# Xinglab/abPOA

Hardware: AMD Instinct MI355X
Metric: read-sets/sec (consensus bit-exact) + DP Gcells/sec (roofline.dp_gcells_per_s) (higher is better)
Workload: dtype int16

## Files before the change

### abpoa_amd/csrc/msa_device.cpp

```cpp
#include <algorithm>
#include <atomic>
#include <chrono>
#include <limits.h>
#include <mutex>
#include <stdio.h>
#include <stdlib.h>
#include <string.h>
#include <thread>
#include <vector>
#include <hip/hip_runtime.h>
#include "engine_options.h"
#include "batch_stream.h"
#include "msa_device.h"
#include "poa_device.h"
#include "poa_graph.h"
#include "dir_plane.h"
#include "msa_batch.h"
#include "msa_device_debug.h"
#include "msa_device_plan.h"
#include "routing.h"

namespace abpoa_hip {

namespace {
// ... 277 lines not shown
    b.left = p.scratch; b.right = p.scratch;
    if (gen_io) {
        b.out_off = p.out_off; b.out_row = p.out_row; b.left = (int32_t *)(dr + L.o_left); b.right = (int32_t *)(dr + L.o_right); b.row_active = dr + L.o_act;
    }
    b.dp_beg_sn = (int32_t *)(dr + L.o_bsn); b.dp_end_sn = (int32_t *)(dr + L.o_esn); b.row_cell_off = (int64_t *)(dr + L.o_coff);
    b.row_max_i = (int32_t *)(dr + L.o_rmi);
    b.planes = C.planes.dev; b.cigar = p.cigar;
    b_rc = b;
    if (pl.amb) {
        b.want_lr = (sc->wb >= 0 && !pl.general) ? 1 : 0;
        b_rc = b; b_rc.want_lr = 0; b_rc.fresh_band = sc->wb >= 0 ? 0 : 1;
    }
    return 0;
}

void plan_rounds(Job &J) {
    const DevicePlan &pl = J.pl; const abpoa_hip_scoring_t *sc = &pl.sc; const PoaDev &p = J.p; const DevBatch &b = J.b; DevBatch &b_r = J.b_r;
    bool &dbg_sync = J.dbg_sync, &use_rounds = J.use_rounds; size_t &rounds_lds = J.rounds_lds;
    dbg_sync = opt_on("ABPOA_HIP_DEVSYNC");
    use_rounds = !pl.local && pl.rounds_possible && !dbg_sync && b.lds.wide_on == 0 && !(b.dbg & 64) && pl.max_reads > 2 && !opt_on("ABPOA_HIP_LOCKSTEP");
    b_r = b; rounds_lds = 0;
    if (use_rounds) {
        auto dyn_of = [&](const DevBatch &x) { return std::max<size_t>(std::max<size_t>((size_t)x.lds.total_rows, (size_t)x.lds.total_tail),
                (size_t)5 * (size_t)(p.lds_rows > 0 ? p.lds_rows : 0)); };
        rounds_lds = dyn_of(b_r);
        int st_lds = 0; int nb = poa_rounds_residency(sc->gap_mode, rounds_lds, &st_lds);
        if (nb < 4 && J.n_sets > nb * 256) {
            const int budget = 160 * 1024 / 4 - st_lds - 512, excess = (int)rounds_lds - budget;
            if (excess > 0 && (size_t)b_r.lds.total_tail == rounds_lds && b_r.lds.bt_bytes_tail - ((excess + 15) & ~15) >= 8 * 1024) {
                b_r.lds.bt_bytes_tail -= (excess + 15) & ~15; b_r.lds.total_tail -= (excess + 15) & ~15;
                rounds_lds = dyn_of(b_r); nb = poa_rounds_residency(sc->gap_mode, rounds_lds, &st_lds);
            }
        }
        b_r.lds.te_on = 0;
        if (b_r.dir_mode && sc->gap_mode != ABPOA_HIP_LINEAR_GAP && !opt_on("ABPOA_HIP_LATE_TAIL")) {
            const int avail = (int)rounds_lds - b_r.lds.phase_off, tables = (SPEC_WK - 1) * SPEC_PM_ROWS * 4;
            const int ring = (b_r.lds.total_rows - b_r.lds.phase_off + 15) & ~15;
            int w_ = ((avail - tables) / SPEC_WK) & ~15, m_ = w_;
            if (w_ < ring) { m_ = ring; w_ = ((avail - tables - m_) / (SPEC_WK - 1)) & ~15; }
            if (w_ >= SPEC_EARLY_MIN) { b_r.lds.te_on = 1; b_r.lds.te_main = m_; b_r.lds.te_w = w_; }
        }
        const int n_cu = device_cu_count(J.device);
        if (nb < 1 || J.n_sets > nb * n_cu) use_rounds = false;
        if (opt_set("ABPOA_HIP_VERBOSE")) fprintf(stderr,
                "[abpoa-hip] all-rounds kernel: %s, %zu B dynamic + %d B static LDS per workgroup, %d workgroups per CU, " "backtrack window %d B, helpers %s (%d + 3 x %d B)\n",
                use_rounds ? "on" : "off", rounds_lds, st_lds, nb, b_r.lds.bt_bytes_tail, b_r.lds.te_on ? "under the row loop" : "after the row loop", b_r.lds.te_main, b_r.lds.te_w);
    }
}

int queue_job(Job &J, DeviceDebug &dbg) {
    const DevicePlan &pl = J.pl; Cache &C = *J.C; const Layout &L = J.L; PoaDev &p = J.p; const DevBatch &b = J.b;
    hipStream_t st = C.stream; uint8_t *hi = C.in.host, *hg = C.graph.host, *dg = C.graph.dev, *dr = C.rows.dev; int rc;
    const int64_t *roff = (const int64_t *)(hi + L.o_roff);
    auto stage = [&](const char *what, int k) { return dbg.stage(what, k); };
    if (pl.gen_io()) HIP_OK(hipMemsetAsync(dr + L.o_act, 1, (size_t)pl.node_tot, st), ABPOA_HIP_ELAUNCH);
    if (pl.amb) HIP_OK(hipMemsetAsync(dg + L.o_isrc, 0, (size_t)pl.tot_reads, st), ABPOA_HIP_ELAUNCH);
    J.t_queue = now_s();
    HIP_OK(hipEventRecord(C.ev[0], st), ABPOA_HIP_ELAUNCH);
    if (stage("upload", 0)) return ABPOA_HIP_ELAUNCH;
    HIP_OK(launch_poa_init(p, st), ABPOA_HIP_ELAUNCH);
    if (stage("init", 0)) return ABPOA_HIP_ELAUNCH;
    dbg.graph_check(0);
    HIP_OK(hipEventRecord(C.ev[1], st), ABPOA_HIP_ELAUNCH);
    for (int k = 1; k < pl.max_reads; ++k) {
        if (k == 2 && !J.rest_up) {
            stage_reads(J, 2, pl.max_reads);
            HIP_OK(hipMemcpyAsync(C.in.dev + L.o_reads + (size_t)J.split_at, hi + L.o_reads + (size_t)J.split_at, (size_t)(roff[pl.tot_reads] - J.split_at),
                    hipMemcpyHostToDevice, C.copy_stream), ABPOA_HIP_ELAUNCH);
            HIP_OK(hipEventRecord(C.ev_copy, C.copy_stream), ABPOA_HIP_ELAUNCH);
            HIP_OK(hipStreamWaitEvent(st, C.ev_copy, 0), ABPOA_HIP_ELAUNCH);
            J.rest_up = true;
        }
        if (J.use_rounds && k == 2) {
            HIP_OK(hipEventRecord(C.ev[2], st), ABPOA_HIP_ELAUNCH);
            HIP_OK(launch_poa_rounds(p, J.b_r, (int32_t *)(dr + L.o_ticket), C.in.host + L.o_rargs, J.slot, 2, J.rounds_lds, st), ABPOA_HIP_ELAUNCH);
            HIP_OK(hipEventRecord(C.ev[3], st), ABPOA_HIP_ELAUNCH);
            break;
        }
        p.round = k;
        hipEvent_t *e = C.ev.data() + 4 * k;
        if (p.order_mode) { HIP_OK(launch_poa_order(p, st), ABPOA_HIP_ELAUNCH); if (stage("row order", k)) return ABPOA_HIP_ELAUNCH; dbg.order_check(k); }
        HIP_OK(launch_poa_prepare(p, st), ABPOA_HIP_ELAUNCH);
        if (stage("prepare", k)) return ABPOA_HIP_ELAUNCH;
        HIP_OK(hipEventRecord(e[0], st), ABPOA_HIP_ELAUNCH);
        if (pl.general) { HIP_OK(launch_dp_general(b, st), ABPOA_HIP_ELAUNCH); HIP_OK(hipEventRecord(e[1], st), ABPOA_HIP_ELAUNCH); }
        else HIP_OK(launch_dp_fast(b, st, e[1]), ABPOA_HIP_ELAUNCH);
        if (stage("dp rows + tail", k)) return ABPOA_HIP_ELAUNCH;
        if (pl.amb) {
            HIP_OK(launch_poa_strand_check(p, st), ABPOA_HIP_ELAUNCH);
            HIP_OK(launch_dp_general(J.b_rc, st), ABPOA_HIP_ELAUNCH);
            HIP_OK(launch_poa_strand_pick(p, st), ABPOA_HIP_ELAUNCH);
            if (stage("strand retry", k)) return ABPOA_HIP_ELAUNCH;
        }
        dbg.balance_report(k, b, e[0], e[1]);
        HIP_OK(hipEventRecord(e[2], st), ABPOA_HIP_ELAUNCH);
        HIP_OK(launch_poa_fuse(p, st), ABPOA_HIP_ELAUNCH);
        if (stage("fuse", k)) return ABPOA_HIP_ELAUNCH;
        dbg.graph_check(k);
        HIP_OK(hipEventRecord(e[3], st), ABPOA_HIP_ELAUNCH);
    }
    if (pl.want_cons) { HIP_OK(launch_poa_consensus(p, st), ABPOA_HIP_ELAUNCH); if (stage("consensus", pl.max_reads)) return ABPOA_HIP_ELAUNCH; }
    if (pl.want_msa) { HIP_OK(launch_poa_msa_rank(p, st), ABPOA_HIP_ELAUNCH); if (stage("msa rank", pl.max_reads)) return ABPOA_HIP_ELAUNCH; }
    HIP_OK(hipMemcpyAsync(hg, dg, J.dl_bytes, hipMemcpyDeviceToHost, st), ABPOA_HIP_ELAUNCH);
    HIP_OK(hipStreamSynchronize(st), ABPOA_HIP_ELAUNCH);
    int64_t msa_total = 0;
    if (pl.want_msa) {
        const PoaState *hs_ = (const PoaState *)(hg + L.o_state);
        J.msa_off.resize(J.n_sets);
        for (int s = 0; s < J.n_sets; ++s) { J.msa_off[s] = msa_total; if (hs_[s].status == POA_ST_OK && hs_[s].n_nodes > 2) msa_total += (int64_t)(J.sets[s].n_reads
                + (pl.want_cons ? 1 : 0)) * std::max(0, hs_[s].msa_len); }
        if (msa_total > 0) {
            if ((rc = C.msa.need_dev((size_t)msa_total)) || (rc = C.msa.need_host((size_t)msa_total))) return rc;
            memcpy(hi + L.o_msaoff_h, J.msa_off.data(), 8 * (size_t)J.n_sets);
            HIP_OK(hipMemcpyAsync(dg + L.o_msaoff, hi + L.o_msaoff_h, 8 * (size_t)J.n_sets, hipMemcpyHostToDevice, st), ABPOA_HIP_ELAUNCH);
            p.msa_out = C.msa.dev;
            HIP_OK(launch_poa_msa_fill(p, st), ABPOA_HIP_ELAUNCH);
            if (stage("msa fill", pl.max_reads)) return ABPOA_HIP_ELAUNCH;
            HIP_OK(hipMemcpyAsync(C.msa.host, C.msa.dev, (size_t)msa_total, hipMemcpyDeviceToHost, st), ABPOA_HIP_ELAUNCH);
            HIP_OK(hipStreamSynchronize(st), ABPOA_HIP_ELAUNCH);
        }
    }
    J.t_done = now_s();
    return 0;
}

void fill_stats(const Job &J, DeviceRunStats *stats) {
    const DevicePlan &pl = J.pl; Cache &C = *J.C; const Layout &L = J.L; const PoaDev &p = J.p;
    if (opt_set("ABPOA_HIP_ORDER_PROF") && p.order_mode) {
        const PoaState *hs_ = (const PoaState *)(C.graph.host + L.o_state); double a_[4] = {0, 0, 0, 0};
        for (int s = 0; s < J.n_sets; ++s) for (int i = 0; i < 4; ++i) a_[i] += (double)hs_[s].t_phase[i];
        fprintf(stderr, "[abpoa-hip] order walk per set: %.0f single-node passes x %.0f ticks, %.0f parallel passes x %.0f ticks\n", a_[2] / J.n_sets,
                a_[2] > 0 ? a_[0] / a_[2] : 0.0, a_[3] / J.n_sets, a_[3] > 0 ? a_[1] / a_[3] : 0.0);
    }
    if (!stats) return;
    float ms = 0;
    hipEvent_t prev = C.ev[1];
    for (int k = 1; k < (J.use_rounds ? 2 : pl.max_reads); ++k) {
        hipEvent_t *e = C.ev.data() + 4 * k;
        (void)hipEventElapsedTime(&ms, prev, e[0]); stats->prepare_ms += ms;
        (void)hipEventElapsedTime(&ms, e[0], e[1]); stats->rows_ms += ms;
        (void)hipEventElapsedTime(&ms, e[1], e[2]); stats->tail_ms += ms;
        (void)hipEventElapsedTime(&ms, e[2], e[3]); stats->fuse_ms += ms;
        prev = e[3];
    }
    if (J.use_rounds) {
        (void)hipEventElapsedTime(&ms, C.ev[2], C.ev[3]); stats->rounds_ms = ms; stats->rounds_launches = 1;
        const PoaState *hs_ = (const PoaState *)(C.graph.host + L.o_state);
        double tp[4] = {0, 0, 0, 0}, tmax = 0; for (int s = 0; s < J.n_sets; ++s) { double t_ = 0;
                if (hs_[s].status == POA_ST_OK) stats->rounds_algo_bytes += hs_[s].algo_bytes - hs_[s].algo_bytes_before;
        for (int i = 0; i < 4; ++i) { tp[i] += (double)hs_[s].t_phase[i]; t_ += (double)hs_[s].t_phase[i]; } tmax = std::max(tmax, t_); }
        const double tall = tp[0] + tp[1] + tp[2] + tp[3];
        if (tall > 0) { stats->prepare_ms += ms * tp[0] / tall; stats->rows_ms += ms * tp[1] / tall; stats->tail_ms += ms * tp[2] / tall;
                stats->fuse_ms += ms * tp[3] / tall;
                        for (int i = 0; i < 4; ++i) stats->rounds_mticks[i] = tp[i] / J.n_sets * 1e-6; stats->rounds_rows_share = tp[1] / tall;
                        stats->rounds_mean_over_max = J.n_sets > 0 && tmax > 0 ? tall / J.n_sets / tmax : 0; }
        if (opt_set("ABPOA_HIP_VERBOSE") && J.n_sets > 0 && tall > 0) {
            static const char *const ph_[4] = {"prepare", "rows", "backtrack", "fuse"};
            std::vector<double> v_((size_t)J.n_sets);
            for (int i = 0; i < 4; ++i) {
                for (int s = 0; s < J.n_sets; ++s) v_[s] = (double)hs_[s].t_phase[i];
                std::sort(v_.begin(), v_.end());
                fprintf(stderr, "[abpoa-hip] all-rounds kernel, M ticks per set, %-9s: mean %.3f  p99 %.3f  max %.3f\n", ph_[i], tp[i] / J.n_sets * 1e-6,
                        v_[(size_t)std::min<long long>(J.n_sets - 1, (long long)J.n_sets * 99 / 100)] * 1e-6, v_[(size_t)J.n_sets - 1] * 1e-6);
            }
            fprintf(stderr, "[abpoa-hip] all-rounds kernel, set totals: mean %.3f M ticks, max %.3f M ticks, max / mean %.3f\n", tall / J.n_sets * 1e-6, tmax * 1e-6,
                    tmax / (tall / J.n_sets));
// ... 120 lines not shown
```

### abpoa_amd/csrc/msa_device_debug.cpp

```cpp
#include <algorithm>
#include <limits.h>
#include <stdio.h>
#include <stdlib.h>
#include <string.h>
#include "engine_options.h"
#include "msa_device_debug.h"

namespace abpoa_hip {

void consensus_flat(int n, const int32_t *order, const uint8_t *base, const uint8_t *nout, const int32_t *out_id, const int32_t *out_w,
                    const int32_t *n_read, std::vector<int> *ids, std::vector<uint8_t> *bases, std::vector<int> *cov, std::vector<int> &score,
                            std::vector<int> &max_out, int out_cap) {
    ids->clear(); bases->clear(); cov->clear();
    if (n <= 2) return;
    score.assign(n, 0); max_out.assign(n, -1);
    for (int r = n - 1; r >= 0; --r) {
        const int cur = order[r];
        const int32_t *oi = out_id + (size_t)cur * out_cap, *ow = out_w + (size_t)cur * out_cap; const int no = nout[cur];
        if (cur == 1) { max_out[cur] = -1; score[cur] = 0; }
        else if (cur == 0) {
            int path_score = -1, path_max_w = -1, max_id = -1;
            for (int i = 0; i < no; ++i) if (ow[i] > path_max_w || (ow[i] == path_max_w && score[oi[i]] > path_score)) { max_id = oi[i]; path_score =
                    score[oi[i]]; path_max_w = ow[i]; }
            max_out[cur] = max_id;
        } else {
            int max_w = INT_MIN, max_id = -1;
            for (int i = 0; i < no; ++i) {
                if (max_w < ow[i]) { max_w = ow[i]; max_id = oi[i]; }
                else if (max_w == ow[i] && score[max_id] <= score[oi[i]]) max_id = oi[i];
            }
            score[cur] = max_w + score[max_id]; max_out[cur] = max_id;
        }
    }
    for (int cur = max_out[0]; cur != 1 && cur >= 0; cur = max_out[cur]) { ids->push_back(cur); bases->push_back(base[cur]); cov->push_back(n_read[cur]); }
}

DeviceDebug::DeviceDebug(const PoaDev *p, const std::vector<PoaSet> *ps, const abpoa_hip_readset_t *sets, int n_sets, int m, int aln_cap, int max_reads,
        bool want_msa,
                         bool amb, hipStream_t stream)
    : p_(p), ps_(ps), sets_(sets), n_sets_(n_sets), m_(m), aln_cap_(aln_cap), max_reads_(max_reads), want_msa_(want_msa), amb_(amb), st_(stream) {
    on_ = opt_on("ABPOA_HIP_DEVSYNC");
    if (on_) { graphs_.resize(std::min(n_sets, 4)); for (size_t i = 0; i < graphs_.size(); ++i) graphs_[i].reset(sets[i].n_reads, want_msa); }
}

int DeviceDebug::stage(const char *what, int k) {
    if (!on_) return 0;
    fprintf(stderr, "[poa-device] round %d: %s queued\n", k, what); fflush(stderr);
    hipError_t e_ = hipStreamSynchronize(st_);
    fprintf(stderr, "[poa-device] round %d: %s -> %s\n", k, what, hipGetErrorString(e_)); fflush(stderr);
    return e_ == hipSuccess ? 0 : 1;
}

void DeviceDebug::order_check(int k) {
    if (!on_) return;
    const PoaDev &p = *p_; const std::vector<PoaSet> &ps = *ps_; const abpoa_hip_readset_t *sets = sets_; const int n_sets = n_sets_, aln_cap = aln_cap_,
            max_reads = max_reads_; const bool amb = amb_;
    std::vector<PoaGraph> &dbg_graphs = graphs_; (void)n_sets; (void)aln_cap; (void)max_reads; (void)amb; (void)ps; (void)sets;
    for (int s = 0; s < (int)dbg_graphs.size(); ++s) {
        if (k >= sets[s].n_reads) continue;
        PoaState hst; (void)hipMemcpy(&hst, (uint8_t *)p.state + sizeof(PoaState) * s, sizeof(hst), hipMemcpyDeviceToHost);
        if (hst.status != POA_ST_OK) { fprintf(stderr, "[poa-device]   set %d round %d: row order: set not ok (status %d reason %d)\n", s, k, hst.status,
                hst.reason); continue; }
        const int n = hst.n_nodes; std::vector<int32_t> order(n), row(n);
        (void)hipMemcpy(order.data(), p.row_node[hst.order_buf] + ps[s].node0, 4 * (size_t)n, hipMemcpyDeviceToHost);
        (void)hipMemcpy(row.data(), p.nd_row + ps[s].node0, 4 * (size_t)n, hipMemcpyDeviceToHost);
        PoaGraph &G = dbg_graphs[s]; int bad = 0;
        try { G.topological_sort(false); } catch (...) { fprintf(stderr, "[poa-device]   set %d round %d: host sort failed\n", s, k); continue; }
        if (G.n_nodes() != n) { fprintf(stderr, "[poa-device]   set %d round %d: row order check FAILED: node count %d vs host %d\n", s, k, n, G.n_nodes());
                continue; }
        for (int r = 0; r < n; ++r) { if (order[r] != G.index_to_node()[r] && bad++ < 6) fprintf(stderr,
                "[poa-device]   set %d round %d: row %d: device node %d, host node %d\n", s, k, r, order[r], G.index_to_node()[r]);
                                      if (order[r] >= 0 && order[r] < n && row[order[r]] != r && bad++ < 6) fprintf(stderr,
                                              "[poa-device]   set %d round %d: nd_row / order mismatch at row %d\n", s, k, r); }
        fprintf(stderr, "[poa-device]   set %d round %d: row order check %s (%d rows)\n", s, k, bad ? "FAILED" : "ok", n);
    }
}

void DeviceDebug::graph_check(int k) {
    if (!on_) return;
    const PoaDev &p = *p_; const std::vector<PoaSet> &ps = *ps_; const abpoa_hip_readset_t *sets = sets_; const int n_sets = n_sets_, aln_cap = aln_cap_,
            max_reads = max_reads_; const bool amb = amb_;
    std::vector<PoaGraph> &dbg_graphs = graphs_; (void)n_sets; (void)aln_cap; (void)max_reads; (void)amb; (void)ps; (void)sets;
    for (int s = 0; s < (int)dbg_graphs.size(); ++s) {
        if (k >= sets[s].n_reads) continue;
        PoaState hst; (void)hipMemcpy(&hst, (uint8_t *)p.state + sizeof(PoaState) * s, sizeof(hst), hipMemcpyDeviceToHost);
        const PoaSet &S = ps[s]; const int n = hst.n_nodes;
        if (k == 0) dbg_graphs[s].add_alignment(sets[s].seqs[0], sets[s].lens[0], nullptr, 0, 0, sets[s].weights ? sets[s].weights[0] : nullptr);
        else {
            AlnOut ao; (void)hipMemcpy(&ao, (uint8_t *)p.out + sizeof(AlnOut) * s, sizeof(ao), hipMemcpyDeviceToHost);
            std::vector<uint64_t> cg(std::max(1, ao.n_cigar)); (void)hipMemcpy(cg.data(), (uint8_t *)p.cigar + 8 * S.cigar_off, 8 * (size_t)ao.n_cigar,
                    hipMemcpyDeviceToHost);
            fprintf(stderr, "[poa-device]   set %d round %d: dp status %d score %d n_cigar %d rows %d; device state status %d reason %d nodes %d\n", s, k,
                    ao.status, ao.best_score, ao.n_cigar, ao.n_rows_done, hst.status, hst.reason, n);
            if (ao.status != 0) continue;
            uint8_t rcf = 0; if (amb) (void)hipMemcpy(&rcf, p.is_rc + S.read0 + k, 1, hipMemcpyDeviceToHost);
            const int ql_ = sets[s].lens[k]; std::vector<uint8_t> rq_; std::vector<int32_t> rw_;
            if (rcf) { rq_.resize(ql_); for (int j = 0; j < ql_; ++j) { const uint8_t c_ = sets[s].seqs[k][ql_ - 1 - j]; rq_[j] = c_ < 4 ? (uint8_t)(3 - c_)
                    : (uint8_t)4; }
                       if (sets[s].weights && sets[s].weights[k]) { rw_.resize(ql_); for (int j = 0; j < ql_; ++j) rw_[j] = sets[s].weights[k][ql_ - 1 - j]; } }
            dbg_graphs[s].add_alignment(rcf ? rq_.data() : sets[s].seqs[k], ql_, cg.data(), ao.n_cigar, k, rcf && !rw_.empty() ? rw_.data() : (sets[s].weights
                    ? sets[s].weights[k] : nullptr));
        }
        if (hst.status != POA_ST_OK) continue;
        std::vector<uint8_t> base(n), nin(n), nout(n), naln(n); std::vector<int32_t> in(n * (int)p.in_cap), outv(n * (int)p.out_cap), outw(n * (int)p.out_cap),
                aln((size_t)n * aln_cap), nread(n), row(n), order(n);
        auto dl = [&](void *dst, const void *pool, size_t elem, size_t per) { (void)hipMemcpy(dst, (const uint8_t *)pool + (size_t)S.node0 * elem * per,
                (size_t)n * elem * per, hipMemcpyDeviceToHost); };
        dl(base.data(), p.nd_base, 1, 1); dl(nin.data(), p.nd_nin, 1, 1); dl(nout.data(), p.nd_nout, 1, 1); dl(naln.data(), p.nd_naln, 1, 1);
        auto dl_list = [&](int32_t *dst, const int32_t *hot, const int32_t *cold, int cap_) {
            std::vector<int32_t> h_((size_t)n * POA_HOT), c_((size_t)n * (cap_ - POA_HOT));
            (void)hipMemcpy(h_.data(), hot + (size_t)S.node0 * POA_HOT, h_.size() * 4, hipMemcpyDeviceToHost);
            (void)hipMemcpy(c_.data(), cold + (size_t)S.node0 * (cap_ - POA_HOT), c_.size() * 4, hipMemcpyDeviceToHost);
            for (int u_ = 0; u_ < n; ++u_) for (int t_ = 0; t_ < cap_; ++t_) dst[(size_t)u_ * cap_ + t_] = t_ < POA_HOT ? h_[(size_t)u_ * POA_HOT + t_]
                    : c_[(size_t)u_ * (cap_ - POA_HOT) + t_ - POA_HOT];
        };
        dl_list(in.data(), p.nd_in, p.nd_inx, (int)p.in_cap); dl_list(outv.data(), p.nd_out, p.nd_outx, (int)p.out_cap); dl_list(outw.data(), p.nd_outw, p.nd_outwx,
                (int)p.out_cap); dl(aln.data(), p.nd_aln, 4, aln_cap);
        dl(nread.data(), p.nd_nread, 4, 1); dl(row.data(), p.nd_row, 4, 1); dl(order.data(), p.row_node[hst.order_buf], 4, 1);
        int bad = 0;
        auto complain = [&](const char *what, int a, int b_) { if (bad++ < 8) fprintf(stderr, "[poa-device]   set %d round %d: %s (%d, %d)\n", s, k, what, a,
                b_); };
        const PoaGraph &G = dbg_graphs[s];
        if (G.n_nodes() != n) complain("node count differs from host graph", n, G.n_nodes());
        for (int r = 0; r < n; ++r) { if (order[r] < 0 || order[r] >= n) { complain("order entry out of range", r, order[r]); continue;
                } if (row[order[r]] != r) complain("nd_row / order mismatch", r, order[r]); }
        for (int u = 0; u < n && u < G.n_nodes(); ++u) {
            const PoaNode &h = G.node(u);
            if (h.base != base[u]) complain("base differs", u, base[u]);
            if (h.in_id.size() != nin[u]) complain("in-degree differs", u, nin[u]);
            else for (int t = 0; t < std::min<int>(nin[u], (int)p.in_cap); ++t) { if (h.in_id[t] != in[u * (int)p.in_cap + t]) complain("in edge differs", u, t);
                    if (row[in[u * (int)p.in_cap
                    + t]] >= row[u]) complain("order violated (pred row >= row)", in[u * (int)p.in_cap + t], u); }
            if (h.out_id.size() != nout[u]) complain("out-degree differs", u, nout[u]);
            else for (int t = 0; t < std::min<int>(nout[u], (int)p.out_cap); ++t) { if (h.out_id[t] != outv[u * (int)p.out_cap + t]) complain("out edge differs", u,
                    t);
                    if (h.out_w[t] != outw[u * (int)p.out_cap + t]) complain("out weight differs", u, t); }
            if (h.aligned.size() != naln[u]) complain("aligned count differs", u, naln[u]);
            else for (int t = 0; t < naln[u]; ++t) if (h.aligned[t] != aln[(size_t)u * aln_cap + t]) complain("aligned node differs", u, t);
            if (h.n_read != nread[u]) complain("n_read differs", u, nread[u]);
        }
        fprintf(stderr, "[poa-device]   set %d round %d: graph check %s (%d nodes)\n", s, k, bad ? "FAILED" : "ok", n);
    }
}

void DeviceDebug::balance_report(int k, const DevBatch &b, hipEvent_t rows_begin, hipEvent_t rows_end) {
    if (!on_ || !opt_set("ABPOA_HIP_IMBAL")) return;
    const PoaDev &p = *p_; const std::vector<PoaSet> &ps = *ps_; const abpoa_hip_readset_t *sets = sets_; const int n_sets = n_sets_, aln_cap = aln_cap_,
            max_reads = max_reads_; const bool amb = amb_;
    std::vector<PoaGraph> &dbg_graphs = graphs_; (void)n_sets; (void)aln_cap; (void)max_reads; (void)amb; (void)ps; (void)sets;
    hipEvent_t e[2] = {rows_begin, rows_end};
    std::vector<double> &tot_set = tot_set_; double &sum_max = sum_max_;
    std::vector<AlnOut> ho(n_sets); (void)hipMemcpy(ho.data(), p.out, sizeof(AlnOut) * n_sets, hipMemcpyDeviceToHost);
    double sd = 0, sb = 0; long long md = 0, mb = 0, ms_ = 0; for (const AlnOut &o_ : ho) { sd += o_.clk_dp; sb += o_.clk_bt; md = std::max<long long>(md,
            o_.clk_dp); mb = std::max<long long>(mb, o_.clk_bt); ms_ = std::max<long long>(ms_, o_.clk_dp + o_.clk_bt); }
    float rows_ms_ = 0; (void)hipEventElapsedTime(&rows_ms_, e[0], e[1]);
    fprintf(stderr,
            "[poa-device] round %d balance: rows mean %.0f max %lld (%.2f ms on the stream, %.2f Gticks/s) | tail "
// ... 112 lines not shown
```

### abpoa_amd/csrc/msa_device_debug.h

```cpp
#pragma once
#include <vector>
#include <hip/hip_runtime.h>
#include "../../include/abpoa_hip.h"
#include "poa_device.h"
#include "poa_graph.h"

namespace abpoa_hip {

void consensus_flat(int n, const int32_t *order, const uint8_t *base, const uint8_t *nout, const int32_t *out_id, const int32_t *out_w, const int32_t *n_read,
                    std::vector<int> *ids, std::vector<uint8_t> *bases, std::vector<int> *cov, std::vector<int> &score, std::vector<int> &max_out, int out_cap);

class DeviceDebug {
public:
    DeviceDebug(const PoaDev *p, const std::vector<PoaSet> *ps, const abpoa_hip_readset_t *sets, int n_sets, int m, int aln_cap, int max_reads, bool want_msa, bool amb,
                hipStream_t stream);
    bool on() const { return on_; }
    int stage(const char *what, int k);
    void order_check(int k);
    void graph_check(int k);
    void balance_report(int k, const DevBatch &b, hipEvent_t rows_begin, hipEvent_t rows_end);
    void msa_check(const PoaState *hs, const abpoa_hip_msa_t *out);
    void consensus_check(const PoaState *hs, const abpoa_hip_msa_t *out);
private:
    bool on_; const PoaDev *p_; const std::vector<PoaSet> *ps_; const abpoa_hip_readset_t *sets_; int n_sets_, m_, aln_cap_, max_reads_; bool want_msa_, amb_; hipStream_t st_;
    std::vector<PoaGraph> graphs_;
    std::vector<double> tot_set_; double sum_max_ = 0;
};

}
```

### abpoa_amd/csrc/poa_device.hip

```cpp
#include <algorithm>
#include <map>
#include <mutex>
#include <utility>
#include "poa_bodies.h"

namespace abpoa_hip {

__global__ void __launch_bounds__(64) poa_init_kernel(const PoaDev p) {
    const int s = blockIdx.x, lane = threadIdx.x;
    if (s >= p.n_sets) return;
    const PoaSet S = p.sets[s];
    PoaState *st = p.state + s;
    if (lane == 0) { st->order_buf = 0; st->n_cells = 0; st->algo_bytes = 0; st->reason = POA_WHY_NONE; st->cons_len = 0; st->msa_len = 0; st->cigar_dig = 0; for (int i = 0; i < 4; ++i) st->t_phase[i] = 0;
            st->algo_bytes_before = 0; }
    if (S.n_reads <= 0) { if (lane == 0) { st->n_nodes = 2; st->status = POA_ST_OK; } return; }
    const int L = p.read_len[S.read0];
    const uint8_t *seq = p.reads + p.read_off[S.read0];
    const int n = L + 2;
    if (n > S.node_cap) { if (lane == 0) { st->n_nodes = 2; st->status = POA_ST_FALLBACK; st->reason = POA_WHY_NODES_AT_INIT; } return; }
    const int64_t N0 = S.node0;
    for (int u = lane; u < n; u += 64) {
        const int i = u - 2;
        p.nd_base[N0 + u] = u >= 2 ? seq[i] : 0;
        p.nd_naln[N0 + u] = 0;
        int nin = 0, nout = 0, in0 = 0, out0 = 0;
        if (u == 0) { nout = 1; out0 = 2; }
        else if (u == 1) { nin = 1; in0 = L + 1; }
        else { nin = 1; in0 = i == 0 ? 0 : u - 1; nout = 1; out0 = i == L - 1 ? 1 : u + 1; }
        p.nd_nin[N0 + u] = (uint8_t)nin; p.nd_nout[N0 + u] = (uint8_t)nout;
        const int32_t *wq = p.wts ? p.wts + p.read_off[S.read0] : nullptr;
        in_slot(p, S, N0 + u, 0) = in0; out_slot(p, S, N0 + u, 0) = out0; outw_slot(p, S, N0 + u, 0) = !wq ? 1 : (u == 0 ? wq[0] : (u == 1 ? 0 : wq[i == L - 1 ? L - 1 : i + 1]));
        p.nd_nread[N0 + u] = nout;
        if (p.rid_words && nout) { for (int w_ = 0; w_ < p.rid_words; ++w_) p.nd_rid[((N0 + u) * p.out_cap) * p.rid_words + w_] = w_ == 0 ? 1ull : 0ull; }
        const int row = u == 0 ? 0 : (u == 1 ? n - 1 : u - 1);
        p.nd_row[N0 + u] = row; p.row_node[0][N0 + row] = u;
    }
    if (lane == 0) { st->n_nodes = n; st->status = POA_ST_OK; }
}

__global__ void __launch_bounds__(GT) poa_prepare_kernel(const PoaDev p) {
    if ((int)blockIdx.x >= p.n_sets) return;
    poa_prepare_body(p, blockIdx.x, p.round);
}
__global__ void __launch_bounds__(GT) poa_fuse_kernel(const PoaDev p) {
    if ((int)blockIdx.x >= p.n_sets) return;
    poa_fuse_body(p, blockIdx.x, p.round);
}

__global__ void __launch_bounds__(GT) poa_strand_check_kernel(const PoaDev p) {
    const int s = blockIdx.x, tid = threadIdx.x, k = p.round;
    if (s >= p.n_sets) return;
    const PoaSet S = p.sets[s];
    if (tid == 0) p.retry[s] = 0;
    AlnDesc d = p.aln[s];
    const AlnOut o = p.out[s];
    const int status = uni(p.state[s].status), flags = uni(d.flags), o_status = uni(o.status), n_cigar = uni(o.n_cigar), qlen = uni(d.qlen), n_rows = uni(d.n_rows), score = uni(o.best_score);
    if (status != POA_ST_OK || k >= S.n_reads || (flags & ALN_SKIP)) return;
    const int lim = qlen < n_rows - 2 ? qlen : n_rows - 2;
    const bool again = o_status == 0 && (double)score < (double)(lim * p.max_mat) * .3333;
    __syncthreads();
    if (!again) { if (tid == 0) p.aln[s].flags = flags | ALN_SKIP; return; }
    const uint64_t *cg = p.cigar + S.cigar_off; uint64_t *cf = p.cigar_fwd + S.cigar_off;
    for (int i = tid; i < n_cigar; i += GT) cf[i] = cg[i];
    const int64_t off = p.read_off[S.read0 + k];
    const uint8_t *q = p.reads + off; uint8_t *rq = p.reads_rc + off;
    for (int j = tid; j < qlen; j += GT) { const uint8_t c = q[qlen - 1 - j]; rq[j] = c < 4 ? (uint8_t)(3 - c) : (uint8_t)4; }
    if (p.wts) for (int j = tid; j < qlen; j += GT) p.wts_rc[off + j] = p.wts[off + qlen - 1 - j];
    if (tid == 0) {
        p.out_fwd[s] = o;
        d.flags = 0; d.query_off = off + (int64_t)(p.reads_rc - p.reads); p.aln[s] = d;
        p.out[s].status = 0; p.out[s].n_cigar = 0; p.out[s].n_cells = 0;
        p.retry[s] = 1;
    }
}
__global__ void __launch_bounds__(GT) poa_strand_pick_kernel(const PoaDev p) {
    const int s = blockIdx.x, tid = threadIdx.x, k = p.round;
    if (s >= p.n_sets || !uni((int)p.retry[s])) return;
    const PoaSet S = p.sets[s];
    const AlnOut rc = p.out[s], fw = p.out_fwd[s];
    const int rc_status = uni(rc.status), rc_score = uni(rc.best_score), fw_score = uni(fw.best_score), fw_cigar = uni(fw.n_cigar);
    __syncthreads();
    if (rc_status != 0) return;
    if (rc_score > fw_score) { if (tid == 0) { p.is_rc[S.read0 + k] = 1; p.out[s].n_cells = rc.n_cells + fw.n_cells; } return; }
    const uint64_t *cf = p.cigar_fwd + S.cigar_off; uint64_t *cg = p.cigar + S.cigar_off;
    for (int i = tid; i < fw_cigar; i += GT) cg[i] = cf[i];
    if (tid == 0) { AlnOut r = fw; r.n_cells += rc.n_cells; p.out[s] = r; }
}

__global__ void __launch_bounds__(64) poa_consensus_kernel(const PoaDev p) {
    const int s = blockIdx.x, lane = threadIdx.x;
    if (s >= p.n_sets) return;
    const PoaSet S = p.sets[s];
    PoaState *st = p.state + s;
    if (st->status != POA_ST_OK) return;
    const int n = st->n_nodes;
    if (n <= 2) { if (lane == 0) st->cons_len = 0; return; }
    const int64_t N0 = S.node0;
    const int32_t *order = p.row_node[st->order_buf] + N0;
    int32_t *score = p.row_remain + N0;
    int32_t *nextrow = p.row_node_id + N0;
    __shared__ int sh_score[64], sh_next[64], sh_node[64];
    for (int t0 = ((n - 1) >> 6) << 6; t0 >= 0; t0 -= 64) {
        const int r = t0 + lane; const bool valid = r < n;
        const int u = valid ? order[r] : 1;
        const int no = valid ? (int)p.nd_nout[N0 + u] : 0;
        int wmax = INT_MIN;
        for (int t = 0; t < no; ++t) wmax = imax_(wmax, outw_slot(p, S, N0 + u, t));
        constexpr int NCAND = 4;
        unsigned long long dep = 0; int ctr[NCAND], csc[NCAND], ncand = 0;
#pragma unroll
        for (int c_ = 0; c_ < NCAND; ++c_) { ctr[c_] = -1; csc[c_] = 0; }
        for (int t = 0; t < no; ++t) if (outw_slot(p, S, N0 + u, t) == wmax) {
            const int tr = p.nd_row[N0 + out_slot(p, S, N0 + u, t)];
            if (tr < t0 + 64) dep |= 1ull << (tr - t0);
#pragma unroll
            for (int c_ = 0; c_ < NCAND; ++c_) if (c_ == ncand) { ctr[c_] = tr; csc[c_] = tr >= t0 + 64 ? ld_fresh(score + tr) : 0; }
            ++ncand;
        }
        bool done = !valid; int my_score = 0, my_next = -1;
        if (valid && no == 0) { done = true; }
        unsigned long long done_mask = __ballot(done);
        sh_score[lane] = 0; sh_next[lane] = -1;
        __syncthreads();
        for (int it = 0; it < 64 && done_mask != ~0ull; ++it) {
            const bool fire = !done && (dep & ~done_mask) == 0;
            if (fire) {
                int best_sc = INT_MIN, best_row = -1; const bool is_src = u == 0;
                if (ncand <= NCAND) {
#pragma unroll
                    for (int c_ = 0; c_ < NCAND; ++c_) if (c_ < ncand) {
                        const int tr = ctr[c_];
                        const int sc_ = tr < t0 + 64 ? sh_score[tr - t0] : csc[c_];
                        if (best_row < 0 || (is_src ? sc_ > best_sc : sc_ >= best_sc)) { best_sc = sc_; best_row = tr; }
                    }
                } else for (int t = 0; t < no; ++t) if (outw_slot(p, S, N0 + u, t) == wmax) {
                    const int tr = p.nd_row[N0 + out_slot(p, S, N0 + u, t)];
                    const int sc_ = tr < t0 + 64 ? sh_score[tr - t0] : ld_fresh(score + tr);
                    if (best_row < 0 || (is_src ? sc_ > best_sc : sc_ >= best_sc)) { best_sc = sc_; best_row = tr; }
                }
                my_score = wmax + best_sc; my_next = best_row; done = true;
                sh_score[lane] = my_score;
            }
            __syncthreads();
            done_mask |= __ballot(fire);
        }
        if (valid) { score[r] = my_score; nextrow[r] = my_next; }
        __syncthreads();
    }
    int cur = ld_fresh(nextrow + 0), len = 0; bool overflow = false;
    const int sink_row = n - 1;
    while (cur >= 0 && cur < sink_row) {
        const int t0 = cur & ~63;
        const int r = t0 + lane;
        sh_next[lane] = r < n ? ld_fresh(nextrow + r) : -1;
        sh_node[lane] = r < n ? order[r] : 0;
        __syncthreads();
        while (cur >= t0 && cur < t0 + 64 && cur < sink_row) {
            const int u = sh_node[cur - t0];
            if (len < S.cons_cap) { if (lane == 0) { p.cons_node[S.cons0 + len] = u; p.cons_base[S.cons0 + len] = p.nd_base[N0 + u]; p.cons_cov[S.cons0 + len] = p.nd_nread[N0 + u]; } }
            else overflow = true;
            ++len;
            cur = sh_next[cur - t0];
        }
        __syncthreads();
    }
    if (lane == 0) { st->cons_len = len; if (overflow) { st->status = POA_ST_FALLBACK; st->reason = POA_WHY_EDGE_SLOTS; } }
}


constexpr int ORD_KEY = 256;
constexpr int ORD_RING = 1024;
extern __shared__ int ord_lds[];
template <bool L> __device__ __forceinline__ int tbl_ld(const PoaDev &p, int32_t *g, int which, int n, int i) { if constexpr (L) return ord_lds[ORD_RING + which * n + i];
        else return ld_fresh(g + (int64_t)which * n + i); }
template <bool L> __device__ __forceinline__ void tbl_st(const PoaDev &p, int32_t *g, int which, int n, int i, int v) { if constexpr (L) ord_lds[ORD_RING + which * n + i] = v;
        else g[(int64_t)which * n + i] = v; }
template <bool L> __device__ __forceinline__ void tbl_dec_max(const PoaDev &p, int32_t *g, int n, int i, int key) {
    if constexpr (L) { atomicSub(&ord_lds[ORD_RING + i], 1); atomicMax(&ord_lds[ORD_RING + n + i], key); }
    else { atomicSub(g + i, 1); atomicMax(g + (int64_t)n + i, key); }
}

template <bool L> __device__ __forceinline__ void tbl_fence() {
    if (L) asm volatile("s_waitcnt lgkmcnt(0)" ::: "memory"); else asm volatile("s_waitcnt vmcnt(0) lgkmcnt(0)" ::: "memory");
    __builtin_amdgcn_wave_barrier();
}
template <bool L>
__device__ __forceinline__ bool poa_order_body(const PoaDev &p, const PoaSet &S, const int n, int32_t *order) {
    const int lane = threadIdx.x;
    const int64_t N0 = S.node0;
    int32_t *g = p.scratch + S.scratch0;
    uint8_t *const s_naln = (uint8_t *)(ord_lds + ORD_RING + 2 * n);
    uint16_t *const s_next = (uint16_t *)(ord_lds + ORD_RING + 2 * n + ((n + 3) >> 2));
    uint16_t *const s_q = s_next + ((n + 1) & ~1);
    const bool QL = L && n < 65535;
    auto qget = [&](int pos_, int head_, int tail_) __attribute__((always_inline)) -> int {
        if (QL) return (int)s_q[pos_];
        if (tail_ - head_ <= ORD_RING) return ord_lds[pos_ & (ORD_RING - 1)];
        return ld_fresh(order + pos_);
    };
    auto qput = [&](int at_, int node_) __attribute__((always_inline)) {
        if (QL) s_q[at_] = (uint16_t)node_;
        else { order[at_] = node_; p.nd_row[N0 + node_] = at_; ord_lds[at_ & (ORD_RING - 1)] = node_; }
    };
    for (int u = lane; u < n; u += 64) {
        tbl_st<L>(p, g, 0, n, u, p.nd_nin[N0 + u]); tbl_st<L>(p, g, 1, n, u, -1);
        if (L) { s_naln[u] = p.nd_naln[N0 + u]; s_next[u] = (p.nd_nout[N0 + u] == 1 && n < 65535) ? (uint16_t)p.nd_out[(N0 + u) * POA_HOT] : (uint16_t)0xffff; }
    }
    auto naln_of = [&](int v) __attribute__((always_inline)) -> int { return L ? (int)s_naln[v] : (int)p.nd_naln[N0 + v]; };
    if (lane == 0) qput(0, 0);
    tbl_fence<L>();
    int head = 0, tail = 1;
#ifdef ABPOA_HIP_ORDER_PROF
    long long t_seq = 0, t_par = 0, n_seq = 0, n_par = 0, t_last = (long long)__builtin_amdgcn_s_memtime();
#define ORD_PROF(T, N) { const long long t_ = (long long)__builtin_amdgcn_s_memtime(); T += t_ - t_last; t_last = t_; ++N; }
#else
#define ORD_PROF(T, N)
#endif
    while (head < tail) {
        if (tail - head == 1) {
            if (!QL && tail - head > ORD_RING) asm volatile("s_waitcnt vmcnt(0)" ::: "memory");
            const int u = uni(qget(head, head, tail));
            int no; int4 o4;
            const int nx = L ? uni((int)s_next[u]) : 0xffff;
            if (nx != 0xffff) { no = 1; o4 = make_int4(nx, 0, 0, 0); }
            else { no = uni((int)p.nd_nout[N0 + u]); o4 = *(const int4 *)(p.nd_out + (N0 + u) * POA_HOT); }
            int at = tail;
            for (int k = 0; k < no; ++k) {
                const int v = uni(k == 0 ? o4.x : (k == 1 ? o4.y : (k == 2 ? o4.z : (k == 3 ? o4.w : out_slot(p, S, N0 + u, k)))));
                const int d = uni(tbl_ld<L>(p, g, 0, n, v)) - 1;
                if (lane == 0) { tbl_st<L>(p, g, 0, n, v, d); tbl_st<L>(p, g, 1, n, v, head * ORD_KEY + k); }
                if (d != 0) continue;
                const int na = uni(naln_of(v));
                bool ready = true;
                if (na > 0) { tbl_fence<L>(); for (int t = 0; t < na && ready; ++t) ready = uni(tbl_ld<L>(p, g, 0, n, p.nd_aln[(N0 + v) * p.aln_cap + t])) == 0; }
                if (!ready) continue;
                if (at + 1 + na > n) return false;
                if (lane == 0) qput(at, v);
                if (lane < na) qput(at + 1 + lane, p.nd_aln[(N0 + v) * p.aln_cap + lane]);
                at += 1 + na;
            }
            tail = at; ++head;
            tbl_fence<L>();
            ORD_PROF(t_seq, n_seq)
            continue;
        }
        const int cnt = imin_(64, tail - head), pos = head + lane; const bool act = lane < cnt;
        int u = 1, no = 0; int4 o4 = make_int4(0, 0, 0, 0);
// ... 307 lines not shown
```

Measured before the change: 20050.

## Pipeline consensus kernel loads and parallelize heaviest-path resolution within a wave

The consensus kernel now prefetches row order, out-edge slots and successor rows three tiles ahead in a software pipeline. It resolves single-candidate chains with shuffle pointer jumping instead of one row per iteration, and replaces block barriers with wave-level fences. Path emission is now parallel across lanes using readlane plus a popcount prefix, with the next tile prefetched. A debug prepare-stage checker is also added. The aim is to cut load latency and serial iterations in consensus, at the cost of more registers and subtle tie-breaking and ordering risks.

```diff
diff --git a/abpoa_amd/csrc/msa_device.cpp b/abpoa_amd/csrc/msa_device.cpp
--- a/abpoa_amd/csrc/msa_device.cpp
+++ b/abpoa_amd/csrc/msa_device.cpp
@@ -383,6 +383,7 @@
         if (p.order_mode) { HIP_OK(launch_poa_order(p, st), ABPOA_HIP_ELAUNCH); if (stage("row order", k)) return ABPOA_HIP_ELAUNCH; dbg.order_check(k); }
         HIP_OK(launch_poa_prepare(p, st), ABPOA_HIP_ELAUNCH);
         if (stage("prepare", k)) return ABPOA_HIP_ELAUNCH;
+        dbg.prepare_check(k);
         HIP_OK(hipEventRecord(e[0], st), ABPOA_HIP_ELAUNCH);
         if (pl.general) { HIP_OK(launch_dp_general(b, st), ABPOA_HIP_ELAUNCH); HIP_OK(hipEventRecord(e[1], st), ABPOA_HIP_ELAUNCH); }
         else HIP_OK(launch_dp_fast(b, st, e[1]), ABPOA_HIP_ELAUNCH);
diff --git a/abpoa_amd/csrc/msa_device_debug.cpp b/abpoa_amd/csrc/msa_device_debug.cpp
--- a/abpoa_amd/csrc/msa_device_debug.cpp
+++ b/abpoa_amd/csrc/msa_device_debug.cpp
@@ -73,6 +73,72 @@
                                       if (order[r] >= 0 && order[r] < n && row[order[r]] != r && bad++ < 6) fprintf(stderr,
                                               "[poa-device]   set %d round %d: nd_row / order mismatch at row %d\n", s, k, r); }
         fprintf(stderr, "[poa-device]   set %d round %d: row order check %s (%d rows)\n", s, k, bad ? "FAILED" : "ok", n);
+    }
+}
+
+void DeviceDebug::prepare_check(int k) {
+    if (!on_) return;
+    const PoaDev &p = *p_; const std::vector<PoaSet> &ps = *ps_;
+    for (int s = 0; s < (int)graphs_.size(); ++s) {
+        if (k >= sets_[s].n_reads) continue;
+        PoaState hst; (void)hipMemcpy(&hst, (uint8_t *)p.state + sizeof(PoaState) * s, sizeof(hst), hipMemcpyDeviceToHost);
+        if (hst.status != POA_ST_OK) continue;
+        const PoaSet &S = ps[s]; const int n = hst.n_nodes;
+        PoaGraph &G = graphs_[s]; int bad = 0;
+        try { G.topological_sort(true); } catch (...) { fprintf(stderr, "[poa-device]   set %d round %d: host sort failed\n", s, k); continue; }
+        if (G.n_nodes() != n) { fprintf(stderr, "[poa-device]   set %d round %d: prepare check FAILED: node count %d vs host %d\n", s, k, n, G.n_nodes()); continue; }
+        std::vector<int32_t> order(n), row(n, -1), rem(n), nid(n), poff(n + 1), ooff; std::vector<uint8_t> base(n), sd(n); std::vector<uint32_t> pd(2 * (size_t)n);
+        bool dl_ok = true;
+        auto dl = [&](void *dst, const void *src, size_t bytes) { if (bytes && hipMemcpy(dst, src, bytes, hipMemcpyDeviceToHost) != hipSuccess) dl_ok = false; };
+        dl(order.data(), p.row_node[hst.order_buf] + S.node0, 4 * (size_t)n); dl(rem.data(), p.row_remain + S.node0, 4 * (size_t)n);
+        dl(nid.data(), p.row_node_id + S.node0, 4 * (size_t)n); dl(poff.data(), p.pred_off + S.node0, 4 * (size_t)(n + 1));
+        dl(base.data(), p.row_base + S.node0, (size_t)n); dl(sd.data(), p.row_sdist + S.node0, (size_t)n); dl(pd.data(), p.row_pd + 2 * S.node0, 8 * (size_t)n);
+        auto complain = [&](const char *what, int r, long long got, long long want) { if (bad++ < 6) fprintf(stderr,
+                "[poa-device]   set %d round %d: row %d: %s %lld, host %lld\n", s, k, r, what, got, want); };
+        bool usable = true;
+        for (int r = 0; r < n; ++r) { if (order[r] < 0 || order[r] >= n || row[order[r]] >= 0) { complain("row order entry", r, order[r], -1); usable = false; } else row[order[r]] = r; }
+        if (usable) {
+            std::vector<int32_t> want_poff(n + 1, 0), want_pred, want_ooff(n + 1, 0), want_out;
+            for (int r = 0; r < n; ++r) {
+                const PoaNode &h = G.node(order[r]);
+                want_poff[r] = (int32_t)want_pred.size(); if (r > 0) for (int t = 0; t < (int)h.in_id.size(); ++t) want_pred.push_back(row[h.in_id[t]]);
+                want_ooff[r] = (int32_t)want_out.size(); for (int t = 0; t < (int)h.out_id.size(); ++t) want_out.push_back(row[h.out_id[t]]);
+            }
+            want_poff[n] = (int32_t)want_pred.size(); want_ooff[n] = (int32_t)want_out.size();
+            std::vector<int32_t> pred(std::max<size_t>(1, want_pred.size())), outr;
+            if ((long long)want_pred.size() <= S.pred_cap) dl(pred.data(), p.pred_row + S.pred0, 4 * want_pred.size());
+            else complain("predecessor entries beyond the set's slots, set still ok:", n, (long long)want_pred.size(), S.pred_cap);
+            if (p.out_off) { ooff.resize(n + 1); dl(ooff.data(), p.out_off + S.node0, 4 * (size_t)(n + 1)); outr.resize(std::max<size_t>(1, want_out.size()));
+                             if ((long long)want_out.size() <= S.pred_cap) dl(outr.data(), p.out_row + S.pred0, 4 * want_out.size()); }
+            for (int r = 0; r < n; ++r) {
+                const int u = order[r]; const PoaNode &h = G.node(u);
+                if (base[r] != h.base) complain("row_base", r, base[r], h.base);
+                if (nid[r] != u) complain("row_node_id", r, nid[r], u);
+                const int want_rem = p.banded ? G.remain()[u] : 0;
+                if (rem[r] != want_rem) complain("remaining length", r, rem[r], want_rem);
+                if (poff[r] != want_poff[r]) complain("pred_off", r, poff[r], want_poff[r]);
+                const int np = want_poff[r + 1] - want_poff[r]; unsigned long long want_pd = ~0ull;
+                for (int t = 0; t < np; ++t) {
+                    const int pr = want_pred[want_poff[r] + t];
+                    if ((long long)want_pred.size() <= S.pred_cap && pred[want_poff[r] + t] != pr) complain("pred_row entry", r, pred[want_poff[r] + t], pr);
+                    if (t < 8 && r - pr <= 254) want_pd = (want_pd & ~(0xffull << (8 * t))) | ((unsigned long long)(r - pr) << (8 * t));
+                }
+                const unsigned long long got_pd = (unsigned long long)pd[2 * (size_t)r] | ((unsigned long long)pd[2 * (size_t)r + 1] << 32);
+                if (got_pd != want_pd) complain("row_pd (low dword shown)", r, (long long)(uint32_t)got_pd, (long long)(uint32_t)want_pd);
+                int far = 0; for (int t = 0; t < (int)h.out_id.size(); ++t) far = std::max(far, row[h.out_id[t]]);
+                const int want_sd = far >= n - 1 ? 255 : std::min(std::max(far - r, 0), 255);
+                if (sd[r] != want_sd) complain("row_sdist", r, sd[r], want_sd);
+                if (p.out_off) {
+                    if (ooff[r] != want_ooff[r]) complain("out_off", r, ooff[r], want_ooff[r]);
+                    if ((long long)want_out.size() <= S.pred_cap) for (int t = want_ooff[r]; t < want_ooff[r + 1]; ++t) if (outr[t] != want_out[t]) complain("out_row entry", r, outr[t], want_out[t]);
+                }
+            }
+            if (poff[n] != want_poff[n]) complain("pred_off[n]", n, poff[n], want_poff[n]);
+            if (p.out_off && ooff[n] != want_ooff[n]) complain("out_off[n]", n, ooff[n], want_ooff[n]);
+        }
+        if (!dl_ok) { fprintf(stderr, "[poa-device]   set %d round %d: prepare check FAILED: download failed\n", s, k); continue; }
+        fprintf(stderr, "[poa-device]   set %d round %d: prepare check %s (%d rows, %d differences)%s\n", s, k, bad ? "FAILED" : "ok", n, bad,
+                p.out_off ? " successor rows too" : "");
     }
 }
 
diff --git a/abpoa_amd/csrc/msa_device_debug.h b/abpoa_amd/csrc/msa_device_debug.h
--- a/abpoa_amd/csrc/msa_device_debug.h
+++ b/abpoa_amd/csrc/msa_device_debug.h
@@ -17,6 +17,7 @@
     bool on() const { return on_; }
     int stage(const char *what, int k);
     void order_check(int k);
+    void prepare_check(int k);
     void graph_check(int k);
     void balance_report(int k, const DevBatch &b, hipEvent_t rows_begin, hipEvent_t rows_end);
     void msa_check(const PoaState *hs, const abpoa_hip_msa_t *out);
diff --git a/abpoa_amd/csrc/poa_device.hip b/abpoa_amd/csrc/poa_device.hip
--- a/abpoa_amd/csrc/poa_device.hip
+++ b/abpoa_amd/csrc/poa_device.hip
@@ -87,6 +87,43 @@
     if (tid == 0) { AlnOut r = fw; r.n_cells += rc.n_cells; p.out[s] = r; }
 }
 
+namespace {
+struct ConsNode {
+    int u = 1, no = 0;
+    int4 w = make_int4(0, 0, 0, 0), o = make_int4(0, 0, 0, 0);
+};
+struct ConsRow {
+    int u = 1, no = 0, wmax = INT_MIN;
+    int hw[POA_HOT] = {0, 0, 0, 0};
+    int rr[POA_HOT] = {-1, -1, -1, -1};
+    int cw[POA_HOT] = {0, 0, 0, 0}, co[POA_HOT] = {0, 0, 0, 0};
+};
+__device__ __forceinline__ ConsNode cons_level2(const PoaDev &p, const int64_t N0, const int u, const bool valid) {
+    ConsNode a; a.u = u;
+    if (valid) {
+        a.no = (int)p.nd_nout[N0 + u];
+        a.w = *(const int4 *)(p.nd_outw + (N0 + u) * POA_HOT);
+        a.o = *(const int4 *)(p.nd_out + (N0 + u) * POA_HOT);
+    }
+    return a;
+}
+__device__ __forceinline__ ConsRow cons_level3(const PoaDev &p, const int64_t N0, const ConsNode &a, const bool valid, const int mid_max) {
+    ConsRow b; b.u = a.u; b.no = valid ? a.no : 0;
+    const int w[POA_HOT] = {a.w.x, a.w.y, a.w.z, a.w.w}, o[POA_HOT] = {a.o.x, a.o.y, a.o.z, a.o.w};
+#pragma unroll
+    for (int t = 0; t < POA_HOT; ++t) { b.hw[t] = w[t]; if (t < a.no) b.wmax = imax_(b.wmax, w[t]); }
+    const bool hot = valid && a.no <= POA_HOT, mid = valid && a.no > POA_HOT && a.no <= mid_max;
+#pragma unroll
+    for (int t = 0; t < POA_HOT; ++t) if ((hot && t < a.no && w[t] == b.wmax) || mid) b.rr[t] = p.nd_row[N0 + o[t]];
+    if (mid) {
+        const int64_t Xc = (N0 + a.u) * (p.out_cap - POA_HOT);
+#pragma unroll
+        for (int t = 0; t < POA_HOT; ++t) if (POA_HOT + t < a.no) { b.cw[t] = p.nd_outwx[Xc + t]; b.co[t] = p.nd_outx[Xc + t]; }
+    }
+    return b;
+}
+__device__ __forceinline__ void cons_fence() { asm volatile("s_waitcnt lgkmcnt(0)" ::: "memory"); __builtin_amdgcn_wave_barrier(); }
+}
 __global__ void __launch_bounds__(64) poa_consensus_kernel(const PoaDev p) {
     const int s = blockIdx.x, lane = threadIdx.x;
     if (s >= p.n_sets) return;
@@ -99,32 +136,95 @@
     const int32_t *order = p.row_node[st->order_buf] + N0;
     int32_t *score = p.row_remain + N0;
     int32_t *nextrow = p.row_node_id + N0;
-    __shared__ int sh_score[64], sh_next[64], sh_node[64];
-    for (int t0 = ((n - 1) >> 6) << 6; t0 >= 0; t0 -= 64) {
-        const int r = t0 + lane; const bool valid = r < n;
-        const int u = valid ? order[r] : 1;
-        const int no = valid ? (int)p.nd_nout[N0 + u] : 0;
-        int wmax = INT_MIN;
-        for (int t = 0; t < no; ++t) wmax = imax_(wmax, outw_slot(p, S, N0 + u, t));
-        constexpr int NCAND = 4;
-        unsigned long long dep = 0; int ctr[NCAND], csc[NCAND], ncand = 0;
+    __shared__ int sh_score[64], sh_above[64];
+    constexpr int NCAND = 4;
+    static_assert(POA_HOT == 4 && NCAND == POA_HOT, "the hot slots are read as one int4 and are the candidates of a row without cold slots");
+    const int top = ((n - 1) >> 6) << 6;
+    const int mid_max = imin_(2 * POA_HOT, p.out_cap);
+    auto in_graph = [&](int r_) { return r_ >= 0 && r_ < n; };
+    int u1 = 1; ConsNode node2; ConsRow row3;
+    sh_above[lane] = 0;
+    for (int h = top + 192; h >= 0; h -= 64) {
+        const ConsRow cur = row3;
+        row3 = cons_level3(p, N0, node2, in_graph(h - 64 + lane), mid_max);
+        node2 = cons_level2(p, N0, u1, in_graph(h - 128 + lane));
+        u1 = in_graph(h - 192 + lane) ? order[h - 192 + lane] : 1;
+        if (h > top) continue;
+        const int u = cur.u, no = cur.no; int wmax = cur.wmax;
+        const int t0 = h, r = t0 + lane; const bool valid = r < n;
+        const bool mid = no > POA_HOT && no <= mid_max;
+        const bool slow = no > POA_HOT && !mid;
+        unsigned long long dep = 0; int ctr[NCAND], csc[NCAND], ncand = 0; bool far = false;
 #pragma unroll
         for (int c_ = 0; c_ < NCAND; ++c_) { ctr[c_] = -1; csc[c_] = 0; }
-        for (int t = 0; t < no; ++t) if (outw_slot(p, S, N0 + u, t) == wmax) {
-            const int tr = p.nd_row[N0 + out_slot(p, S, N0 + u, t)];
-            if (tr < t0 + 64) dep |= 1ull << (tr - t0);
-#pragma unroll
-            for (int c_ = 0; c_ < NCAND; ++c_) if (c_ == ncand) { ctr[c_] = tr; csc[c_] = tr >= t0 + 64 ? ld_fresh(score + tr) : 0; }
-            ++ncand;
-        }
-        bool done = !valid; int my_score = 0, my_next = -1;
-        if (valid && no == 0) { done = true; }
+        if (mid) {
+#pragma unroll
+            for (int t = 0; t < POA_HOT; ++t) if (POA_HOT + t < no) wmax = imax_(wmax, cur.cw[t]);
+        }
+        if (!slow) {
+#pragma unroll
+            for (int t = 0; t < POA_HOT; ++t) if (cur.rr[t] >= 0 && (!mid || cur.hw[t] == wmax)) {
+#pragma unroll
+                for (int c_ = 0; c_ < NCAND; ++c_) if (c_ == ncand) ctr[c_] = cur.rr[t];
+                ++ncand;
+            }
+            if (mid) {
+#pragma unroll
+                for (int t = 0; t < POA_HOT; ++t) if (POA_HOT + t < no && cur.cw[t] == wmax) {
+                    const int tr = p.nd_row[N0 + cur.co[t]];
+                    if (tr < t0 + 64) dep |= 1ull << (tr - t0);
+#pragma unroll
+                    for (int c_ = 0; c_ < NCAND; ++c_) if (c_ == ncand) ctr[c_] = tr;
+                    ++ncand;
+                }
+                if (ncand > NCAND) far = true;
+            }
+#pragma unroll
+            for (int c_ = 0; c_ < NCAND; ++c_) if (c_ < ncand) {
+                if (ctr[c_] < t0 + 64) dep |= 1ull << (ctr[c_] - t0);
+                else if (ctr[c_] < t0 + 128) csc[c_] = sh_above[ctr[c_] - t0 - 64];
+                else far = true;
+            }
+        }
+        if (__any(slow || far)) {
+            asm volatile("s_waitcnt vmcnt(0)" ::: "memory");
+            if (slow) {
+                wmax = INT_MIN;
+                for (int t = 0; t < no; ++t) wmax = imax_(wmax, outw_slot(p, S, N0 + u, t));
+                for (int t = 0; t < no; ++t) if (outw_slot(p, S, N0 + u, t) == wmax) {
+                    const int tr = p.nd_row[N0 + out_slot(p, S, N0 + u, t)];
+                    if (tr < t0 + 64) dep |= 1ull << (tr - t0);
+#pragma unroll
+                    for (int c_ = 0; c_ < NCAND; ++c_) if (c_ == ncand) { ctr[c_] = tr; csc[c_] = tr >= t0 + 64 ? ld_fresh(score + tr) : 0; }
+                    ++ncand;
+                }
+            } else if (far) {
+#pragma unroll
+                for (int c_ = 0; c_ < NCAND; ++c_) if (c_ < ncand && ctr[c_] >= t0 + 128) csc[c_] = ld_fresh(score + ctr[c_]);
+            }
+        }
+        bool done = !valid || no == 0; int val = 0, my_next = -1;
+        const bool simple = valid && !slow && ncand == 1;
+        int acc = wmax, tgt = simple ? ctr[0] : r;
+        if (simple) { my_next = ctr[0]; if (ctr[0] >= t0 + 64) { val = wmax + csc[0]; done = true; } }
+        if (__any(simple && !done)) {
+#pragma unroll
+            for (int it = 0; it < 6; ++it) {
+                const bool jump = simple && !done;
+                const int src = jump ? tgt - t0 : lane;
+                const int t_tgt = shfl(tgt, src), t_acc = shfl(acc, src), t_val = shfl(val, src), t_st = shfl((int)done | ((int)jump << 1), src);
+                if (jump) { if (t_st & 1) { val = acc + t_val; done = true; } else if (t_st & 2) { acc += t_acc; tgt = t_tgt; } }
+            }
+        }
+        if (simple && !done) dep = 1ull << (tgt - t0);
+        int my_score = val;
         unsigned long long done_mask = __ballot(done);
-        sh_score[lane] = 0; sh_next[lane] = -1;
-        __syncthreads();
+        sh_score[lane] = val;
+        cons_fence();
         for (int it = 0; it < 64 && done_mask != ~0ull; ++it) {
             const bool fire = !done && (dep & ~done_mask) == 0;
-            if (fire) {
+            if (fire && simple) { my_score = acc + sh_score[tgt - t0]; done = true; sh_score[lane] = my_score; }
+            else if (fire) {
                 int best_sc = INT_MIN, best_row = -1; const bool is_src = u == 0;
                 if (ncand <= NCAND) {
 #pragma unroll
@@ -141,28 +241,35 @@
                 my_score = wmax + best_sc; my_next = best_row; done = true;
                 sh_score[lane] = my_score;
             }
-            __syncthreads();
+            cons_fence();
             done_mask |= __ballot(fire);
         }
         if (valid) { score[r] = my_score; nextrow[r] = my_next; }
-        __syncthreads();
-    }
-    int cur = ld_fresh(nextrow + 0), len = 0; bool overflow = false;
+        sh_above[lane] = my_score;
+        cons_fence();
+    }
+    asm volatile("s_waitcnt vmcnt(0)" ::: "memory");
+    int cur = uni(ld_fresh(nextrow + 0)), len = 0; bool overflow = false;
     const int sink_row = n - 1;
+    int pf_t0 = -1, pf_next = -1, pf_node = 0;
     while (cur >= 0 && cur < sink_row) {
         const int t0 = cur & ~63;
         const int r = t0 + lane;
-        sh_next[lane] = r < n ? ld_fresh(nextrow + r) : -1;
-        sh_node[lane] = r < n ? order[r] : 0;
-        __syncthreads();
+        int nx, nd;
+        if (t0 == pf_t0) { nx = pf_next; nd = pf_node; }
+        else { nx = r < n ? ld_fresh(nextrow + r) : -1; nd = r < n ? order[r] : 0; }
+        unsigned long long on_path = 0;
         while (cur >= t0 && cur < t0 + 64 && cur < sink_row) {
-            const int u = sh_node[cur - t0];
-            if (len < S.cons_cap) { if (lane == 0) { p.cons_node[S.cons0 + len] = u; p.cons_base[S.cons0 + len] = p.nd_base[N0 + u]; p.cons_cov[S.cons0 + len] = p.nd_nread[N0 + u]; } }
-            else overflow = true;
-            ++len;
-            cur = sh_next[cur - t0];
-        }
-        __syncthreads();
+            on_path |= 1ull << (cur - t0);
+            const int to = __builtin_amdgcn_readlane(nx, cur - t0);
+            cur = to > cur ? to : -1;
+        }
+        pf_t0 = t0 + 64;
+        pf_next = r + 64 < n ? ld_fresh(nextrow + r + 64) : -1; pf_node = r + 64 < n ? order[r + 64] : 0;
+        const int at = len + __popcll(on_path & ((1ull << lane) - 1ull));
+        if ((on_path >> lane & 1ull) && at < S.cons_cap) { p.cons_node[S.cons0 + at] = nd; p.cons_base[S.cons0 + at] = p.nd_base[N0 + nd]; p.cons_cov[S.cons0 + at] = p.nd_nread[N0 + nd]; }
+        len += __popcll(on_path);
+        if (len > S.cons_cap) overflow = true;
     }
     if (lane == 0) { st->cons_len = len; if (overflow) { st->status = POA_ST_FALLBACK; st->reason = POA_WHY_EDGE_SLOTS; } }
 }
```

Result: faster. 20340 (median of 6 runs) (+1.4%).
